# achinastone/Tensorium

Hardware: AMD Instinct MI355X
Metric: fp32 SGEMM GFLOP/s (M=N=K=4096) + YOLOv3 conv-fwd images/s (higher is better)
Workload: dtype fp32; 1 GPU; sgemm_nn_4096x4096x4096; M=4096, N=4096, K=4096, parallelism=1 independent replicas, one process per GPU, no data-path collective

## Files before the change

### tensorium_amd/csrc/conv_slab.hip

```cpp
#include <algorithm>
#include <type_traits>

#include "tns_act.hpp"
#include "tns_internal.hpp"

namespace tns {
namespace {

typedef float floatx4 __attribute__((ext_vector_type(4)));

__device__ __forceinline__ void slab_dma16(const float* sbase, unsigned voff, unsigned lds) {
  unsigned keep;
  asm volatile(
      "s_mov_b32 %0, m0\n\ts_mov_b32 m0, %3\n\ts_nop 0\n\t"
      "global_load_lds_dwordx4 %1, %2\n\ts_mov_b32 m0, %0"
      : "=&s"(keep)
      : "v"(voff), "s"(sbase), "s"(lds)
      : "memory");
}

struct SlabFillArgs {
  const float* x;
  int64_t strideX;
  float* slab;
  int C, H, W, stride, pad, dil, ow, ohw, N, K, KT;
  float inv_ohw, inv_ow;
  unsigned bytes;
  int64_t units;
};

__device__ __forceinline__ int slab_div(int n, int d, float inv) {
  int qq = (int)((float)n * inv);
  while (qq * d > n) --qq;
  while ((qq + 1) * d <= n) ++qq;
  return qq;
}

template <int KS, int BK, int BN>
__global__ __launch_bounds__(256) void slab_fill_kernel(SlabFillArgs a) {
  constexpr int NG = BK / 16, KK = KS * KS;
  const int64_t x = (int64_t)blockIdx.x * 256 + threadIdx.x;
  if (x >= a.units) return;
  const int c = (int)(x % BN);
  const int64_t r1 = x / BN;
  const int g = (int)(r1 % NG);
  const int64_t r2 = r1 / NG;
  const int t = (int)(r2 % a.KT), ct = (int)(r2 / a.KT);
  const int n = ct * BN + c;
  float v[16];
  const __amdgpu_buffer_rsrc_t rsrc =
      __builtin_amdgcn_make_buffer_rsrc(const_cast<float*>(a.x), 0, a.bytes, 0x00020000);
  {
    const int nn = n < a.N ? n : a.N - 1;
    const int img = slab_div(nn, a.ohw, a.inv_ohw), pix = nn - img * a.ohw;
    const int oy = slab_div(pix, a.ow, a.inv_ow), ox = pix - oy * a.ow;
    const int iy0 = oy * a.stride - a.pad, ix0 = ox * a.stride - a.pad;
    const int HW = a.H * a.W;
    unsigned mask = 0;
    int toff[KK];
#pragma unroll
    for (int kr = 0; kr < KS; ++kr)
#pragma unroll
      for (int kc = 0; kc < KS; ++kc) {
        const int iy = iy0 + kr * a.dil, ix = ix0 + kc * a.dil;
        mask |= (unsigned)(((unsigned)iy < (unsigned)a.H) & ((unsigned)ix < (unsigned)a.W))
                << (kr * KS + kc);
        toff[kr * KS + kc] = 4 * (kr * a.dil * a.W + kc * a.dil);
      }
    if (n >= a.N) mask = 0;
    const unsigned base = 4u * (unsigned)(img * (int)a.strideX + iy0 * a.W + ix0);
    const int k0 = t * BK + 16 * g;
    int ch = k0 / KK, tap = k0 - ch * KK;
#pragma unroll
    for (int e = 0; e < 16; ++e) {
      int off = toff[0];
#pragma unroll
      for (int u = 1; u < KK; ++u) off = tap == u ? toff[u] : off;
      const unsigned o = ((mask >> tap) & 1u) ? base + 4u * (unsigned)(ch * HW) + (unsigned)off
                                              : 0x80000000u;
      v[e] = __builtin_bit_cast(float, __builtin_amdgcn_raw_buffer_load_b32(rsrc, o, 0, 0));
      if (++tap == KK) {
        tap = 0;
        ++ch;
      }
    }
  }
  float* dst = a.slab + ((r2 * NG + g) * 4 * BN + c) * 4;
#pragma unroll
  for (int q = 0; q < 4; ++q)
    *reinterpret_cast<floatx4*>(dst + q * BN * 4) = floatx4{v[q], v[4 + q], v[8 + q], v[12 + q]};
}

template <int KS, int BK, int BN>
__global__ __launch_bounds__((BN + 63) / 64 * 64) void slab_fill_u_kernel(SlabFillArgs a) {
  constexpr int NG = BK / 16, KK = KS * KS;
  const int c = threadIdx.x;
  if (c >= BN) return;
  const int64_t r1 = blockIdx.x;
  const int g = (int)(r1 % NG);
  const int64_t r2 = r1 / NG;
  const int t = (int)(r2 % a.KT), ct = (int)(r2 / a.KT);
  const int n = ct * BN + c;
  float v[16];
  const __amdgpu_buffer_rsrc_t rsrc =
      __builtin_amdgcn_make_buffer_rsrc(const_cast<float*>(a.x), 0, a.bytes, 0x00020000);
  {
    const int nn = n < a.N ? n : a.N - 1;
    const int img = slab_div(nn, a.ohw, a.inv_ohw), pix = nn - img * a.ohw;
    const int oy = slab_div(pix, a.ow, a.inv_ow), ox = pix - oy * a.ow;
    const int iy0 = oy * a.stride - a.pad, ix0 = ox * a.stride - a.pad;
    const int HW = a.H * a.W;
    unsigned mask = 0;
#pragma unroll
    for (int kr = 0; kr < KS; ++kr)
#pragma unroll
      for (int kc = 0; kc < KS; ++kc) {
        const int iy = iy0 + kr * a.dil, ix = ix0 + kc * a.dil;
        mask |= (unsigned)(((unsigned)iy < (unsigned)a.H) & ((unsigned)ix < (unsigned)a.W))
                << (kr * KS + kc);
      }
    if (n >= a.N) mask = 0;
    const unsigned base = 4u * (unsigned)(img * (int)a.strideX + iy0 * a.W + ix0);
    const int k0 = __builtin_amdgcn_readfirstlane(t * BK + 16 * g);
    int ch = k0 / KK, tap = k0 - ch * KK;
    int kr = tap / KS, kc = tap - kr * KS;
#pragma unroll
    for (int e = 0; e < 16; ++e) {
      const unsigned uoff = 4u * (unsigned)(ch * HW + kr * a.dil * a.W + kc * a.dil);
      const unsigned o = ((mask >> tap) & 1u) ? base + uoff : 0x80000000u;
      v[e] = __builtin_bit_cast(float, __builtin_amdgcn_raw_buffer_load_b32(rsrc, o, 0, 0));
      ++tap;
      if (++kc == KS) {
        kc = 0;
        ++kr;
      }
      if (tap == KK) {
        tap = 0;
        kr = 0;
        ++ch;
      }
    }
  }
  float* dst = a.slab + ((r2 * NG + g) * 4 * BN + c) * 4;
#pragma unroll
  for (int q = 0; q < 4; ++q)
    *reinterpret_cast<floatx4*>(dst + q * BN * 4) = floatx4{v[q], v[4 + q], v[8 + q], v[12 + q]};
}

struct SlabGemmArgs {
  const float* A;
  const float* slab;
  float* C;
  const float* bias;
  int M, N, K, KT, tiles_m, ohw, act;
  bool fuse;
};

template <int BM_, int BN_, int BK_, int WM_, int WN_, int JA_, int NA_, int NS_, int DG_ = 0,
          int MAP_ = 0>
struct SG {
  static constexpr int BM = BM_, BN = BN_, BK = BK_, WM = WM_, WN = WN_, JA = JA_, NA = NA_;
  static constexpr int NS = NS_;
  static constexpr int DG = DG_, MAP = MAP_;
  static constexpr int NW = WM * WN, NT = 64 * NW, J = BN / 16, NG = BK / 16, ROWS = BK / 4;
  static constexpr int JB = NA < WN ? (J - NA * JA) / (WN - NA) : 0;
  static constexpr int A_TILE = ROWS * BM * 4, B_TILE = ROWS * BN * 4, STAGE = A_TILE + B_TILE;
  static constexpr int AU = BM * BK / 4 / NT;
  static constexpr int BDMA = 4 * BK * BN / 1024;
  static constexpr int DPW = (BDMA + NW - 1) / NW;
  static_assert(BM == 16 * WM && BN % 16 == 0 && BK % 16 == 0, "geometry");
  static_assert(NA * JA + (WN - NA) * JB == J && NA >= 1 && NA <= WN, "wave column split");
  static_assert(AU >= 1 && BM * BK / 4 % NT == 0, "A units");
  static_assert(4 * BK * BN % 1024 == 0, "whole DMA instructions");
  static_assert(NS >= 2 && NS * STAGE * 4 <= 163840, "LDS");
  static_assert(NG >= 2 && NG % 2 == 0, "groups: f0 holds group 0 at every tile start");
  static_assert(DPW * (NS - 2) <= 63 && DPW <= 63, "vmcnt immediates");
};

template <int JW>
struct SFrag {
  floatx4 a, b[JW];
};

template <int N>
__device__ __forceinline__ void wait_vm(bool keep_n) {
  if (keep_n)
    asm volatile("s_waitcnt vmcnt(%0)" ::"n"(N) : "memory");
  else
    asm volatile("s_waitcnt vmcnt(0)" ::: "memory");
}

template <class G>
__global__ __launch_bounds__(G::NT, 1) void slab_gemm_kernel(SlabGemmArgs p) {
  constexpr int BM = G::BM, BN = G::BN, BK = G::BK, NG = G::NG, NS = G::NS;
  constexpr int A_TILE = G::A_TILE, STAGE = G::STAGE, AU = G::AU, DPW = G::DPW;
  __shared__ __attribute__((aligned(16))) float smem[NS * STAGE];
  const int tid = threadIdx.x, lane = tid & 63;
  const int w = __builtin_amdgcn_readfirstlane(tid >> 6), wm = w % G::WM, wn = w / G::WM;
  const int r16 = lane & 15, q = lane >> 4;
  int tm, tn;
  {
    const int nb = gridDim.x, bid = blockIdx.x;
    const int xcd = bid & 7, qq = nb >> 3, rr = nb & 7;
    const int wg = (xcd < rr ? xcd * (qq + 1) : rr * (qq + 1) + (xcd - rr) * qq) + (bid >> 3);
    if constexpr (G::MAP == 1) {
      const int tiles_n = (p.N + BN - 1) / BN;
      tn = wg % tiles_n;
      tm = wg / tiles_n;
    } else {
      tm = wg % p.tiles_m;
      tn = wg / p.tiles_m;
    }
  }
  const int m0 = tm * BM, n0 = tn * BN;
  const int N = p.N, K = p.K, nt = p.KT;
  const float* slabT = p.slab + (int64_t)tn * K * BN;
  const unsigned lds0 = (unsigned)(uintptr_t)(__attribute__((address_space(3))) float*)smem;
  const unsigned voff = 16u * (unsigned)lane;
  auto dma_b = [&](int t, int st, int v) {
    if constexpr (G::DG & 1) return;
    int u = w + G::NW * v;
    if (G::BDMA % G::NW != 0 && u >= G::BDMA) u -= G::NW;
    slab_dma16(slabT + (int64_t)t * (BK * BN) + 256 * u, voff,
               lds0 + 4u * (unsigned)(st * STAGE + A_TILE) + 1024u * (unsigned)u);
  };
  auto dma_all = [&](int t, int st) {
#pragma unroll
    for (int v = 0; v < DPW; ++v) dma_b(t, st, v);
  };
  unsigned a_off[AU];
  int a_dst[AU];
#pragma unroll
  for (int u = 0; u < AU; ++u) {
    const int idx = tid + G::NT * u;
    const int lo = idx & 7, rest = idx >> 3;
    const int m = rest % BM, kq4 = lo + 8 * (rest / BM);
    a_off[u] = 4u * (unsigned)(m * K + 4 * kq4);
    a_dst[u] = (4 * (kq4 >> 2)) * BM * 4 + m * 4 + (kq4 & 3);
  }
  const float* a_row0 = p.A + (int64_t)m0 * K;
  floatx4 ra[AU];
  auto load_a = [&](int t) {
    if constexpr (G::DG & 2) return;
    const float* sb = a_row0 + t * BK;
#pragma unroll
    for (int u = 0; u < AU; ++u)
      asm volatile("global_load_dwordx4 %0, %1, %2" : "=v"(ra[u]) : "v"(a_off[u]), "s"(sb) : "memory");
  };
  auto store_a = [&](int st) {
    if constexpr (G::DG & 2) return;
    float* as = smem + st * STAGE;
#pragma unroll
    for (int u = 0; u < AU; ++u) {
      asm volatile("" : "+v"(ra[u]));
      as[a_dst[u]] = ra[u][0];
      as[a_dst[u] + BM * 4] = ra[u][1];
      as[a_dst[u] + 2 * BM * 4] = ra[u][2];
      as[a_dst[u] + 3 * BM * 4] = ra[u][3];
    }
  };

  auto run = [&](auto JWC, const int coff) {
    constexpr int JW = decltype(JWC)::value;
    floatx4 acc[JW];
#pragma unroll
    for (int j = 0; j < JW; ++j) acc[j] = floatx4{0.f, 0.f, 0.f, 0.f};
    using Frag = SFrag<JW>;
    auto frag = [&](int st, int g, Frag& f) {
      const float* ap = smem + st * STAGE + ((4 * g + q) * BM + wm * 16 + r16) * 4;
      f.a = *reinterpret_cast<const floatx4*>(ap);
      const float* bp = smem + st * STAGE + A_TILE + ((4 * g + q) * BN + coff * 16 + r16) * 4;
#pragma unroll
      for (int j = 0; j < JW; ++j) f.b[j] = *reinterpret_cast<const floatx4*>(bp + 64 * j);
    };
    auto mma = [&](const Frag& f) {
#pragma unroll
      for (int i = 0; i < 4; ++i)
#pragma unroll
        for (int j = 0; j < JW; ++j)
          acc[j] = __builtin_amdgcn_mfma_f32_16x16x4f32(f.a[i], f.b[j][i], acc[j], 0, 0, 0);
    };
    auto mma_dma = [&](const Frag& f, int tb, int st) {
      constexpr int NM = 4 * JW, STEP = NM / DPW > 0 ? NM / DPW : 1;
#pragma unroll
      for (int x = 0; x < NM; ++x) {
        const int i = x / JW, j = x % JW;
        acc[j] = __builtin_amdgcn_mfma_f32_16x16x4f32(f.a[i], f.b[j][i], acc[j], 0, 0, 0);
        if (x % STEP == 0 && x / STEP < DPW) dma_b(tb, st, x / STEP);
        __builtin_amdgcn_sched_barrier(0);
      }
      if constexpr (NM / STEP < DPW) {
#pragma unroll
        for (int v = NM / STEP; v < DPW; ++v) dma_b(tb, st, v);
      }
    };

    Frag f0, f1;
    load_a(0);
#pragma unroll
    for (int t = 0; t < NS; ++t) {
      if (t == 1 && nt > 1) {
        wait_vm<0>(false);
        store_a(0);
        load_a(1);
      }
      if (t < nt) dma_all(t, t);
    }
    if (nt == 1) {
      wait_vm<0>(false);
      store_a(0);
    } else {
      if (nt >= NS)
        asm volatile("s_waitcnt vmcnt(%0)" ::"n"(AU + (NS - 1) * DPW) : "memory");
      else
        wait_vm<0>(false);
    }
    __syncthreads();
    frag(0, 0, f0);
    for (int t = 0; t < nt; ++t) {
      const int cur = t % NS;
#pragma unroll
      for (int g = 0; g + 1 < NG; ++g) {
        Frag& fc = (g & 1) ? f1 : f0;
        Frag& fn = (g & 1) ? f0 : f1;
        frag(cur, g + 1, fn);
        __builtin_amdgcn_sched_barrier(0);
        mma(fc);
        __builtin_amdgcn_sched_barrier(0);
      }
      if (t + 1 < nt) {
        const int nxt = (t + 1) % NS;
        if constexpr (NS == 2)
          wait_vm<0>(false);
        else
          wait_vm<DPW>(t + NS - 1 < nt);
        store_a(nxt);
        if constexpr (!(G::DG & 4))
          __syncthreads();
        frag(nxt, 0, f0);
        if (t + 2 < nt) load_a(t + 2);
        __builtin_amdgcn_sched_barrier(0);
        if (t + NS < nt)
          mma_dma(f1, t + NS, cur);
        else
          mma(f1);
      } else {
        mma(f1);
      }
    }

    const int row0 = m0 + wm * 16 + 4 * q;
    float bias[4];
#pragma unroll
    for (int e = 0; e < 4; ++e) bias[e] = p.fuse ? p.bias[row0 + e] : 0.0f;
#pragma unroll
    for (int j = 0; j < JW; ++j) {
      const int n = n0 + coff * 16 + 16 * j + r16;
      if (n >= N) continue;
      const int img = n / p.ohw, pix = n - img * p.ohw;
      float* cp = p.C + ((int64_t)img * p.M + row0) * p.ohw + pix;
#pragma unroll
      for (int e = 0; e < 4; ++e) {
        float v = acc[j][e];
        if (p.fuse) v = act_apply_cheap(v + bias[e], p.act);
        cp[(int64_t)e * p.ohw] = v;
      }
    }
  };
  if constexpr (G::NA == G::WN) {
    run(std::integral_constant<int, G::JA>{}, wn * G::JA);
  } else {
    if (wn < G::NA)
      run(std::integral_constant<int, G::JA>{}, wn * G::JA);
    else
      run(std::integral_constant<int, G::JB>{}, G::NA * G::JA + (wn - G::NA) * G::JB);
  }
}

struct SlabForm {
  int bm, bn, bk;
  hipError_t (*gemm)(const SlabGemmArgs&, hipStream_t);
  hipError_t (*fill)(const SlabFillArgs&, int ks, hipStream_t);
  const char* name;
};

template <class G>
hipError_t launch_slab_gemm(const SlabGemmArgs& a, hipStream_t s) {
  const int64_t blocks = (int64_t)(a.M / G::BM) * ((a.N + G::BN - 1) / G::BN);
  hipLaunchKernelGGL((slab_gemm_kernel<G>), dim3((unsigned)blocks), dim3(G::NT), 0, s, a);
  return hipGetLastError();
}

template <int BK, int BN>
hipError_t launch_slab_fill(const SlabFillArgs& a, int ks, hipStream_t s) {
#ifndef TNS_SLAB_FILL_LANE
  {
    constexpr int NT = (BN + 63) / 64 * 64;
    const int64_t nb = a.units / BN;
    if (nb > 0x7fffffffLL) return hipErrorInvalidValue;
    if (ks == 3)
      hipLaunchKernelGGL((slab_fill_u_kernel<3, BK, BN>), dim3((unsigned)nb), dim3(NT), 0, s, a);
    else if (ks == 1)
      hipLaunchKernelGGL((slab_fill_u_kernel<1, BK, BN>), dim3((unsigned)nb), dim3(NT), 0, s, a);
    else
      return hipErrorInvalidValue;
    return hipGetLastError();
  }
#endif
  const unsigned blocks = (unsigned)((a.units + 255) / 256);
  if (ks == 3)
    hipLaunchKernelGGL((slab_fill_kernel<3, BK, BN>), dim3(blocks), dim3(256), 0, s, a);
  else if (ks == 1)
    hipLaunchKernelGGL((slab_fill_kernel<1, BK, BN>), dim3(blocks), dim3(256), 0, s, a);
  else
    return hipErrorInvalidValue;
  return hipGetLastError();
}

#define TNS_SLAB(BMv, BNv, BKv, WMv, WNv, JAv, NAv, NSv)                                       \
  {BMv, BNv, BKv, launch_slab_gemm<SG<BMv, BNv, BKv, WMv, WNv, JAv, NAv, NSv>>,                   \
   launch_slab_fill<BKv, BNv>,                                                                   \
   "conv_slab<" #BMv "x" #BNv "x" #BKv ",w" #WMv "x" #WNv ",j" #JAv "x" #NAv ",s" #NSv ">"}
#define TNS_SLABD(BMv, BNv, BKv, WMv, WNv, JAv, NAv, NSv, DGv, MAPv)                             \
  {BMv, BNv, BKv, launch_slab_gemm<SG<BMv, BNv, BKv, WMv, WNv, JAv, NAv, NSv, DGv, MAPv>>,       \
   launch_slab_fill<BKv, BNv>,                                                                   \
   "conv_slab<" #BMv "x" #BNv "x" #BKv ",w" #WMv "x" #WNv ",j" #JAv "x" #NAv ",s" #NSv ",dg" #DGv \
   ",map" #MAPv ">"}
const SlabForm kSlab[] = {
    TNS_SLAB(32, 176, 64, 2, 4, 3, 3, 3),
    TNS_SLAB(64, 176, 32, 4, 2, 6, 1, 3),
    TNS_SLAB(64, 176, 32, 4, 2, 6, 1, 4),
    TNS_SLAB(32, 176, 64, 2, 4, 3, 3, 2),
    TNS_SLAB(64, 176, 64, 4, 2, 6, 1, 2),
    TNS_SLAB(32, 176, 32, 2, 2, 6, 1, 4),
    TNS_SLABD(32, 176, 64, 2, 4, 3, 3, 2, 0, 1),
    TNS_SLABD(64, 176, 64, 4, 2, 6, 1, 2, 0, 1),
};
#undef TNS_SLAB
#undef TNS_SLABD
constexpr int kNumSlab = sizeof(kSlab) / sizeof(kSlab[0]);

}

int conv_slab_count() { return kNumSlab; }
const char* conv_slab_name(int v) { return v >= 0 && v < kNumSlab ? kSlab[v].name : ""; }

int conv_slab_pick(int64_t M, int64_t N, int64_t K, int64_t ks) {
  if (ks != 3 || K % 64) return -1;
  if (M == 1024 && N >= 1024) return 3;
  if (M == 512 && N >= 4096) return 4;
  return -1;
}

int64_t conv_slab_floats(int v, int64_t N, int64_t K) {
  if (v < 0 || v >= kNumSlab) return -1;
  const int64_t bn = kSlab[v].bn;
  return (N + bn - 1) / bn * bn * K;
}

hipError_t launch_conv_slab(int v, const ConvSlabArgs& c, float* slab, hipStream_t s) {
  if (v < 0 || v >= kNumSlab) return hipErrorInvalidValue;
  const SlabForm& f = kSlab[v];
  const int64_t N = c.batch * c.ohw;
  if (c.M % f.bm || c.K % f.bk || (c.ks != 1 && c.ks != 3) || N >= (1LL << 22) ||
      4 * c.batch * c.C * c.H * c.W > 0x7fffffffLL ||
      c.K > 0x7fffffffLL / f.bn || (reinterpret_cast<uintptr_t>(c.weights) & 15) || c.K % 4 ||
      (reinterpret_cast<uintptr_t>(slab) & 15) || c.M * c.K > 0x7fffffffLL)
    return hipErrorInvalidValue;
  const int64_t CT = (N + f.bn - 1) / f.bn, KT = c.K / f.bk;
  if (CT * (c.M / f.bm) > 0x7fffffffLL) return hipErrorInvalidValue;
  SlabFillArgs fa{};
  fa.x = c.input; fa.strideX = c.C * c.H * c.W; fa.slab = slab;
  fa.C = (int)c.C; fa.H = (int)c.H; fa.W = (int)c.W; fa.stride = (int)c.stride;
  fa.pad = (int)c.pad; fa.dil = (int)c.dil; fa.ow = (int)c.ow; fa.ohw = (int)c.ohw;
  fa.N = (int)N; fa.K = (int)c.K; fa.KT = (int)KT;
  fa.inv_ohw = (float)((1.0 + 1.0 / 1048576.0) / (double)c.ohw);
  fa.inv_ow = (float)((1.0 + 1.0 / 1048576.0) / (double)c.ow);
  fa.bytes = (unsigned)(4 * c.batch * c.C * c.H * c.W);
  fa.units = CT * KT * (f.bk / 16) * f.bn;
  if (hipError_t e = f.fill(fa, (int)c.ks, s)) return e;
  SlabGemmArgs ga{};
  ga.A = c.weights; ga.slab = slab; ga.C = c.out; ga.bias = c.bias;
  ga.M = (int)c.M; ga.N = (int)N; ga.K = (int)c.K; ga.KT = (int)KT;
  ga.tiles_m = (int)(c.M / f.bm); ga.ohw = (int)c.ohw; ga.act = c.act; ga.fuse = c.bias != nullptr;
  return f.gemm(ga, s);
}

}
```

Measured before the change: 149,000 GFLOP/s.

## Add unrolled two-stage main loop with precomputed LDS addresses for slab conv GEMM

Adds an LP variant of the slab conv GEMM kernel whose main loop is manually unrolled two tiles at a time, with compile-time stage indices, precomputed LDS addresses, pointer-bumped global sources and a clumped six-DMA inline-asm issue for B tiles. The picked slab forms (indices 3 and 4) are switched to this LP=1 variant and the originals are moved to the end of the table. The goal is to cut per-iteration address arithmetic, modulo stage selection and scalar overhead in the conv GEMM's k-loop, at the cost of more code and hand-written register constraints. It also adds optional memtime stamps for profiling, off by default.

Measured after the change: 148,900 GFLOP/s. Within noise of the previous version (-0.0%).

```diff
diff --git a/tensorium_amd/csrc/conv_slab.hip b/tensorium_amd/csrc/conv_slab.hip
--- a/tensorium_amd/csrc/conv_slab.hip
+++ b/tensorium_amd/csrc/conv_slab.hip
@@ -18,6 +18,39 @@
       : "v"(voff), "s"(sbase), "s"(lds)
       : "memory");
 }
+
+template <unsigned STRIDE>
+__device__ __forceinline__ void slab_dma_clump6(const float* sbase, const unsigned (&voff)[6],
+                                                unsigned m0_0, unsigned m0_5) {
+  unsigned keep;
+  asm volatile(
+      "s_mov_b32 %0, m0\n\t"
+      "s_mov_b32 m0, %8\n\ts_nop 0\n\tglobal_load_lds_dwordx4 %1, %7\n\t"
+      "s_add_u32 m0, %8, %10\n\ts_nop 0\n\tglobal_load_lds_dwordx4 %2, %7\n\t"
+      "s_add_u32 m0, %8, %11\n\ts_nop 0\n\tglobal_load_lds_dwordx4 %3, %7\n\t"
+      "s_add_u32 m0, %8, %12\n\ts_nop 0\n\tglobal_load_lds_dwordx4 %4, %7\n\t"
+      "s_add_u32 m0, %8, %13\n\ts_nop 0\n\tglobal_load_lds_dwordx4 %5, %7\n\t"
+      "s_mov_b32 m0, %9\n\ts_nop 0\n\tglobal_load_lds_dwordx4 %6, %7\n\t"
+      "s_mov_b32 m0, %0"
+      : "=&s"(keep)
+      : "v"(voff[0]), "v"(voff[1]), "v"(voff[2]), "v"(voff[3]), "v"(voff[4]), "v"(voff[5]),
+        "s"(sbase), "s"(m0_0), "s"(m0_5), "n"(STRIDE), "n"(2 * STRIDE), "n"(3 * STRIDE),
+        "n"(4 * STRIDE)
+      : "memory", "scc");
+}
+
+#ifdef TNS_SLAB_STAMPS
+#define TNS_SLAB_STAMP(i)                                          \
+  do {                                                             \
+    const unsigned long long n_ = __builtin_amdgcn_s_memtime();    \
+    sacc[i] += n_ - slast;                                         \
+    slast = n_;                                                    \
+  } while (0)
+#else
+#define TNS_SLAB_STAMP(i) \
+  do {                    \
+  } while (0)
+#endif
 
 struct SlabFillArgs {
   const float* x;
@@ -154,14 +187,17 @@
   const float* bias;
   int M, N, K, KT, tiles_m, ohw, act;
   bool fuse;
+#ifdef TNS_SLAB_STAMPS
+  unsigned long long* stamps;
+#endif
 };
 
 template <int BM_, int BN_, int BK_, int WM_, int WN_, int JA_, int NA_, int NS_, int DG_ = 0,
-          int MAP_ = 0>
+          int MAP_ = 0, int LP_ = 0>
 struct SG {
   static constexpr int BM = BM_, BN = BN_, BK = BK_, WM = WM_, WN = WN_, JA = JA_, NA = NA_;
   static constexpr int NS = NS_;
-  static constexpr int DG = DG_, MAP = MAP_;
+  static constexpr int DG = DG_, MAP = MAP_, LP = LP_;
   static constexpr int NW = WM * WN, NT = 64 * NW, J = BN / 16, NG = BK / 16, ROWS = BK / 4;
   static constexpr int JB = NA < WN ? (J - NA * JA) / (WN - NA) : 0;
   static constexpr int A_TILE = ROWS * BM * 4, B_TILE = ROWS * BN * 4, STAGE = A_TILE + B_TILE;
@@ -175,6 +211,7 @@
   static_assert(NS >= 2 && NS * STAGE * 4 <= 163840, "LDS");
   static_assert(NG >= 2 && NG % 2 == 0, "groups: f0 holds group 0 at every tile start");
   static_assert(DPW * (NS - 2) <= 63 && DPW <= 63, "vmcnt immediates");
+  static_assert(LP == 0 || NS == 2, "the unrolled loop: two stages");
 };
 
 template <int JW>
@@ -198,6 +235,9 @@
   const int tid = threadIdx.x, lane = tid & 63;
   const int w = __builtin_amdgcn_readfirstlane(tid >> 6), wm = w % G::WM, wn = w / G::WM;
   const int r16 = lane & 15, q = lane >> 4;
+#ifdef TNS_SLAB_STAMPS
+  unsigned long long sacc[5] = {0, 0, 0, 0, 0}, slast = 0;
+#endif
   int tm, tn;
   {
     const int nb = gridDim.x, bid = blockIdx.x;
@@ -245,7 +285,10 @@
     const float* sb = a_row0 + t * BK;
 #pragma unroll
     for (int u = 0; u < AU; ++u)
-      asm volatile("global_load_dwordx4 %0, %1, %2" : "=v"(ra[u]) : "v"(a_off[u]), "s"(sb) : "memory");
+      asm volatile("global_load_dwordx4 %0, %1, %2"
+                   : "=v"(ra[u])
+                   : "v"(a_off[u]), "s"(sb)
+                   : "memory");
   };
   auto store_a = [&](int st) {
     if constexpr (G::DG & 2) return;
@@ -296,56 +339,225 @@
     };
 
     Frag f0, f1;
-    load_a(0);
-#pragma unroll
-    for (int t = 0; t < NS; ++t) {
-      if (t == 1 && nt > 1) {
+    if constexpr (G::LP == 0) {
+      load_a(0);
+#pragma unroll
+      for (int t = 0; t < NS; ++t) {
+        if (t == 1 && nt > 1) {
+          wait_vm<0>(false);
+          store_a(0);
+          load_a(1);
+        }
+        if (t < nt) dma_all(t, t);
+      }
+      if (nt == 1) {
         wait_vm<0>(false);
         store_a(0);
-        load_a(1);
-      }
-      if (t < nt) dma_all(t, t);
-    }
-    if (nt == 1) {
-      wait_vm<0>(false);
-      store_a(0);
+      } else {
+        if (nt >= NS)
+          asm volatile("s_waitcnt vmcnt(%0)" ::"n"(AU + (NS - 1) * DPW) : "memory");
+        else
+          wait_vm<0>(false);
+      }
+      __syncthreads();
+      frag(0, 0, f0);
+#ifdef TNS_SLAB_STAMPS
+      slast = __builtin_amdgcn_s_memtime();
+#endif
+      for (int t = 0; t < nt; ++t) {
+        const int cur = t % NS;
+        TNS_SLAB_STAMP(0);
+#pragma unroll
+        for (int g = 0; g + 1 < NG; ++g) {
+          Frag& fc = (g & 1) ? f1 : f0;
+          Frag& fn = (g & 1) ? f0 : f1;
+          frag(cur, g + 1, fn);
+          __builtin_amdgcn_sched_barrier(0);
+          mma(fc);
+          __builtin_amdgcn_sched_barrier(0);
+        }
+        TNS_SLAB_STAMP(1);
+        if (t + 1 < nt) {
+          const int nxt = (t + 1) % NS;
+          if constexpr (NS == 2)
+            wait_vm<0>(false);
+          else
+            wait_vm<DPW>(t + NS - 1 < nt);
+          store_a(nxt);
+          TNS_SLAB_STAMP(2);
+          if constexpr (!(G::DG & 4))
+            __syncthreads();
+          TNS_SLAB_STAMP(3);
+          frag(nxt, 0, f0);
+          if (t + 2 < nt) load_a(t + 2);
+          __builtin_amdgcn_sched_barrier(0);
+          if (t + NS < nt)
+            mma_dma(f1, t + NS, cur);
+          else
+            mma(f1);
+        } else {
+          mma(f1);
+        }
+        TNS_SLAB_STAMP(4);
+      }
     } else {
-      if (nt >= NS)
-        asm volatile("s_waitcnt vmcnt(%0)" ::"n"(AU + (NS - 1) * DPW) : "memory");
-      else
-        wait_vm<0>(false);
-    }
-    __syncthreads();
-    frag(0, 0, f0);
-    for (int t = 0; t < nt; ++t) {
-      const int cur = t % NS;
-#pragma unroll
-      for (int g = 0; g + 1 < NG; ++g) {
-        Frag& fc = (g & 1) ? f1 : f0;
-        Frag& fn = (g & 1) ? f0 : f1;
-        frag(cur, g + 1, fn);
+      typedef __attribute__((address_space(3))) floatx4 LdsV4;
+      typedef __attribute__((address_space(3))) float LdsF;
+      unsigned fa[2], fb[2], sa[2][AU];
+#pragma unroll
+      for (int st = 0; st < 2; ++st) {
+        fa[st] = lds0 + 4u * (unsigned)(st * STAGE + (q * BM + wm * 16 + r16) * 4);
+        fb[st] = lds0 + 4u * (unsigned)(st * STAGE + A_TILE + (q * BN + coff * 16 + r16) * 4);
+        asm volatile("" : "+v"(fa[st]), "+v"(fb[st]));
+#pragma unroll
+        for (int u = 0; u < AU; ++u) {
+          sa[st][u] = lds0 + 4u * (unsigned)(st * STAGE + a_dst[u]);
+          asm volatile("" : "+v"(sa[st][u]));
+        }
+      }
+      auto fragc = [&](auto STC, auto GC, Frag& f) __attribute__((always_inline)) {
+        constexpr int ST = decltype(STC)::value, g = decltype(GC)::value;
+        f.a = *(const LdsV4*)(fa[ST] + 64u * g * BM);
+#pragma unroll
+        for (int j = 0; j < JW; ++j) f.b[j] = *(const LdsV4*)(fb[ST] + 64u * g * BN + 256u * j);
+      };
+      const float* asrc = a_row0;
+      auto load_an = [&]() __attribute__((always_inline)) {
+        if constexpr (!(G::DG & 2)) {
+#pragma unroll
+          for (int u = 0; u < AU; ++u)
+            asm volatile("global_load_dwordx4 %0, %1, %2"
+                         : "=v"(ra[u])
+                         : "v"(a_off[u]), "s"(asrc)
+                         : "memory");
+        }
+        asrc += BK;
+      };
+      auto store_an = [&](auto STC) __attribute__((always_inline)) {
+        constexpr int ST = decltype(STC)::value;
+        if constexpr (G::DG & 2) return;
+#pragma unroll
+        for (int u = 0; u < AU; ++u) {
+#pragma unroll
+          for (int i = 0; i < 4; ++i) *(LdsF*)(sa[ST][u] + 16u * i * BM) = ra[u][i];
+        }
+      };
+      auto wait_all = [&]() __attribute__((always_inline)) {
+        if constexpr (G::DG & 2) {
+          asm volatile("s_waitcnt vmcnt(0)" ::: "memory");
+        } else {
+          static_assert(AU == 1 || AU == 2, "A units named by the wait");
+          if constexpr (AU == 1)
+            asm volatile("s_waitcnt vmcnt(0)" : "+v"(ra[0])::"memory");
+          else
+            asm volatile("s_waitcnt vmcnt(0)" : "+v"(ra[0]), "+v"(ra[1])::"memory");
+        }
+      };
+      const float* bsrc = slabT + 256 * w;
+      unsigned bvo[DPW], bm0[2], bm0l[2];
+      int ul = w + G::NW * (DPW - 1);
+      if (G::BDMA % G::NW != 0 && ul >= G::BDMA) ul -= G::NW;
+#pragma unroll
+      for (int v = 0; v < DPW; ++v)
+        bvo[v] = voff + 1024u * (unsigned)(v < DPW - 1 ? G::NW * v : ul - w);
+#pragma unroll
+      for (int st = 0; st < 2; ++st) {
+        bm0[st] = lds0 + 4u * (unsigned)(st * STAGE + A_TILE) + 1024u * (unsigned)w;
+        bm0l[st] = lds0 + 4u * (unsigned)(st * STAGE + A_TILE) + 1024u * (unsigned)ul;
+      }
+      auto dma_one = [&](auto STC, int v) __attribute__((always_inline)) {
+        constexpr int ST = decltype(STC)::value;
+        slab_dma16(bsrc, bvo[v], v == DPW - 1 ? bm0l[ST] : bm0[ST] + 1024u * G::NW * (unsigned)v);
+      };
+      auto dma_tile = [&](auto STC) __attribute__((always_inline)) {
+        constexpr int ST = decltype(STC)::value;
+        if constexpr (!(G::DG & 1)) {
+          if constexpr (DPW == 6) {
+            slab_dma_clump6<1024u * G::NW>(bsrc, bvo, bm0[ST], bm0l[ST]);
+          } else {
+#pragma unroll
+            for (int v = 0; v < DPW; ++v) dma_one(STC, v);
+          }
+        }
+        bsrc += BK * BN;
+      };
+      auto tile = [&](auto STC, auto KDC) __attribute__((always_inline)) {
+        constexpr int ST = decltype(STC)::value, KD = decltype(KDC)::value;
+        constexpr std::integral_constant<int, ST ^ 1> NXC{};
+        TNS_SLAB_STAMP(0);
+        if constexpr (KD >= 1) load_an();
+        fragc(STC, std::integral_constant<int, 1>{}, f1);
         __builtin_amdgcn_sched_barrier(0);
-        mma(fc);
+        mma(f0);
         __builtin_amdgcn_sched_barrier(0);
-      }
-      if (t + 1 < nt) {
-        const int nxt = (t + 1) % NS;
-        if constexpr (NS == 2)
-          wait_vm<0>(false);
-        else
-          wait_vm<DPW>(t + NS - 1 < nt);
-        store_a(nxt);
-        if constexpr (!(G::DG & 4))
-          __syncthreads();
-        frag(nxt, 0, f0);
-        if (t + 2 < nt) load_a(t + 2);
-        __builtin_amdgcn_sched_barrier(0);
-        if (t + NS < nt)
-          mma_dma(f1, t + NS, cur);
-        else
+        if constexpr (NG == 4) {
+          fragc(STC, std::integral_constant<int, 2>{}, f0);
+          __builtin_amdgcn_sched_barrier(0);
           mma(f1);
+          __builtin_amdgcn_sched_barrier(0);
+          fragc(STC, std::integral_constant<int, 3>{}, f1);
+          __builtin_amdgcn_sched_barrier(0);
+          mma(f0);
+          __builtin_amdgcn_sched_barrier(0);
+        }
+        TNS_SLAB_STAMP(1);
+        if constexpr (KD >= 1) {
+          wait_all();
+          store_an(NXC);
+          TNS_SLAB_STAMP(2);
+          if constexpr (!(G::DG & 4))
+            __syncthreads();
+          TNS_SLAB_STAMP(3);
+          fragc(NXC, std::integral_constant<int, 0>{}, f0);
+          if constexpr (KD == 2) {
+            __builtin_amdgcn_sched_barrier(0);
+#pragma unroll
+            for (int x = 0; x < 4 * JW; ++x) {
+              const int i = x / JW, j = x % JW;
+              acc[j] = __builtin_amdgcn_mfma_f32_16x16x4f32(f1.a[i], f1.b[j][i], acc[j], 0, 0, 0);
+              if (x == JW - 1) {
+                __builtin_amdgcn_sched_barrier(0);
+                dma_tile(STC);
+                __builtin_amdgcn_sched_barrier(0);
+              }
+            }
+          } else {
+            __builtin_amdgcn_sched_barrier(0);
+            mma(f1);
+          }
+        } else {
+          mma(f1);
+        }
+        TNS_SLAB_STAMP(4);
+      };
+      constexpr std::integral_constant<int, 0> C0{};
+      constexpr std::integral_constant<int, 1> C1{};
+      constexpr std::integral_constant<int, 2> C2{};
+      static_assert(NG == 4 || NG == 2, "groups of the unrolled tile");
+      load_an();
+      dma_tile(C0);
+      wait_all();
+      store_an(C0);
+      if (nt > 1) dma_tile(C1);
+      __syncthreads();
+      fragc(C0, C0, f0);
+#ifdef TNS_SLAB_STAMPS
+      slast = __builtin_amdgcn_s_memtime();
+#endif
+      int t = 0;
+      for (; t + 3 < nt; t += 2) {
+        tile(C0, C2);
+        tile(C1, C2);
+      }
+      if (t + 2 < nt) {
+        tile(C0, C2);
+        tile(C1, C1);
+        tile(C0, C0);
+      } else if (nt > 1) {
+        tile(C0, C1);
+        tile(C1, C0);
       } else {
-        mma(f1);
+        tile(C0, C0);
       }
     }
 
@@ -375,7 +587,21 @@
     else
       run(std::integral_constant<int, G::JB>{}, G::NA * G::JA + (wn - G::NA) * G::JB);
   }
-}
+#ifdef TNS_SLAB_STAMPS
+  if (lane == 0 && p.stamps != nullptr && blockIdx.x < (1u << 14)) {
+    unsigned long long* d = p.stamps + ((size_t)blockIdx.x * G::NW + w) * 8;
+#pragma unroll
+    for (int i = 0; i < 5; ++i) d[i] = sacc[i];
+    d[5] = (unsigned long long)nt;
+    d[6] = (unsigned long long)w;
+    d[7] = (unsigned long long)(wn < G::NA ? G::JA : G::JB);
+  }
+#endif
+}
+
+#ifdef TNS_SLAB_STAMPS
+unsigned long long* g_slab_stamps = nullptr;
+#endif
 
 struct SlabForm {
   int bm, bn, bk;
@@ -426,16 +652,24 @@
    launch_slab_fill<BKv, BNv>,                                                                   \
    "conv_slab<" #BMv "x" #BNv "x" #BKv ",w" #WMv "x" #WNv ",j" #JAv "x" #NAv ",s" #NSv ",dg" #DGv \
    ",map" #MAPv ">"}
+#define TNS_SLABL(BMv, BNv, BKv, WMv, WNv, JAv, NAv, NSv, LPv)                                   \
+  {BMv, BNv, BKv, launch_slab_gemm<SG<BMv, BNv, BKv, WMv, WNv, JAv, NAv, NSv, 0, 0, LPv>>,        \
+   launch_slab_fill<BKv, BNv>,                                                                   \
+   "conv_slab<" #BMv "x" #BNv "x" #BKv ",w" #WMv "x" #WNv ",j" #JAv "x" #NAv ",s" #NSv ",lp" #LPv \
+   ">"}
 const SlabForm kSlab[] = {
     TNS_SLAB(32, 176, 64, 2, 4, 3, 3, 3),
     TNS_SLAB(64, 176, 32, 4, 2, 6, 1, 3),
     TNS_SLAB(64, 176, 32, 4, 2, 6, 1, 4),
-    TNS_SLAB(32, 176, 64, 2, 4, 3, 3, 2),
-    TNS_SLAB(64, 176, 64, 4, 2, 6, 1, 2),
+    TNS_SLABL(32, 176, 64, 2, 4, 3, 3, 2, 1),
+    TNS_SLABL(64, 176, 64, 4, 2, 6, 1, 2, 1),
     TNS_SLAB(32, 176, 32, 2, 2, 6, 1, 4),
     TNS_SLABD(32, 176, 64, 2, 4, 3, 3, 2, 0, 1),
     TNS_SLABD(64, 176, 64, 4, 2, 6, 1, 2, 0, 1),
+    TNS_SLAB(32, 176, 64, 2, 4, 3, 3, 2),
+    TNS_SLAB(64, 176, 64, 4, 2, 6, 1, 2),
 };
+#undef TNS_SLABL
 #undef TNS_SLAB
 #undef TNS_SLABD
 constexpr int kNumSlab = sizeof(kSlab) / sizeof(kSlab[0]);
@@ -483,7 +717,17 @@
   ga.A = c.weights; ga.slab = slab; ga.C = c.out; ga.bias = c.bias;
   ga.M = (int)c.M; ga.N = (int)N; ga.K = (int)c.K; ga.KT = (int)KT;
   ga.tiles_m = (int)(c.M / f.bm); ga.ohw = (int)c.ohw; ga.act = c.act; ga.fuse = c.bias != nullptr;
+#ifdef TNS_SLAB_STAMPS
+  ga.stamps = g_slab_stamps;
+#endif
   return f.gemm(ga, s);
 }
 
-}
+#ifdef TNS_SLAB_STAMPS
+extern "C" int tns_debug_slab_stamps(unsigned long long* dev_buf) {
+  g_slab_stamps = dev_buf;
+  return 0;
+}
+#endif
+
+}
```
